# tprodanov/locityper

Hardware: AMD Instinct MI355X
Metric: reads/s through the whole genotyping path (scored + prefiltered + default solver scheme); reads_scored_per_s and genotypes_solved_per_s give the two halves (higher is better)
Workload: dtype f64

## Files before the change

locityper_amd/csrc/lcty_api.hip:

```cpp
#include <algorithm>
#include <cmath>
#include <memory>
#include <numeric>

#include "lcty_objects.hpp"

using namespace lcty;

namespace lcty {
static thread_local std::string g_last_error;
thread_local hipStream_t tl_stream = nullptr;
void set_last_error(const std::string& msg) { g_last_error = msg; }
}

hipEvent_t lcty_ctx::get_event() {
    hipEvent_t e;
    if (!event_pool.empty()) { e = event_pool.back(); event_pool.pop_back(); return e; }
    LCTY_HIP(hipEventCreate(&e));
    return e;
}

void lcty_ctx::fold_oldest(lcty::KernelTimer& t, size_t count) {
    count = std::min(count, t.pending.size());
    for (size_t i = 0; i < count; i++) {
// ... 51 lines not shown
        int n = 0;
        if (hipGetDeviceCount(&n) != hipSuccess || n == 0) {
            (void)hipGetLastError();
            fail(LCTY_ERR_RUNTIME, "no HIP device is visible: liblocityper_hip has no CPU fallback");
        }
        if (device_id < 0 || device_id >= n) fail(LCTY_ERR_INVALID_INPUT, "device %d out of range (0..%d)", device_id, n - 1);
        auto c = std::unique_ptr<lcty_ctx>(new lcty_ctx());
        c->device = device_id;
        LCTY_HIP(hipSetDevice(device_id));
        LCTY_HIP(hipGetDeviceProperties(&c->props, device_id));
        LCTY_HIP(hipStreamCreateWithFlags(&c->stream.main, hipStreamNonBlocking));
        *out = c.release();
    });
}

void lcty_ctx_destroy(lcty_ctx* ctx) {
    if (!ctx) return;
    (void)hipSetDevice(ctx->device);
    (void)hipStreamSynchronize(ctx->stream);
    for (auto& t : ctx->timers) for (auto& pr : t.pending) { (void)hipEventDestroy(pr.first); (void)hipEventDestroy(pr.second); }
    for (auto e : ctx->event_pool) (void)hipEventDestroy(e);
    if (ctx->gate.ev) (void)hipEventDestroy(ctx->gate.ev);
    if (ctx->gate.init_ev) (void)hipEventDestroy(ctx->gate.init_ev);
    if (ctx->side) { (void)hipStreamSynchronize(ctx->side); (void)hipStreamDestroy(ctx->side); }
    if (ctx->fore) { (void)hipStreamSynchronize(ctx->fore); (void)hipStreamDestroy(ctx->fore); }
    for (auto& slot : ctx->given_slots) if (slot->stream) { (void)hipStreamSynchronize(slot->stream); (void)hipStreamDestroy(slot->stream); }
    (void)hipStreamDestroy(ctx->stream.main);
    delete ctx;
}

int32_t lcty_ctx_synchronize(lcty_ctx* ctx) {
    return guarded([&] {
        if (!ctx) fail(LCTY_ERR_INVALID_INPUT, "null argument");
        ctx->activate();
        LCTY_HIP(hipStreamSynchronize(ctx->stream));
        if (ctx->side) LCTY_HIP(hipStreamSynchronize(ctx->side));
    });
}

int32_t lcty_host_alloc(lcty_ctx* ctx, uint64_t bytes, void** out) {
    return guarded([&] {
        if (!ctx || !out) fail(LCTY_ERR_INVALID_INPUT, "null argument");
        ctx->activate();
        *out = nullptr;
        LCTY_HIP(hipHostMalloc(out, std::max<uint64_t>(bytes, 1), hipHostMallocDefault));
    });
// ... 290 lines not shown
```

locityper_amd/csrc/lcty_common.hpp:

```cpp
#pragma once

#include <hip/hip_runtime.h>

#include <cstdarg>
#include <cstdint>
#include <cstdio>
#include <cstring>
#include <map>
#include <memory>
#include <condition_variable>
#include <mutex>
#include <stdexcept>
#include <string>
#include <vector>

#include "../../include/locityper_hip.h"

namespace lcty {

#ifdef LCTY_DIAG
constexpr bool kDiag = true;
#else
constexpr bool kDiag = false;
#endif
// ... 129 lines not shown
        if (!on) on = stream;
        lcty::KernelTimer& t = timers[kernel];
        hipEvent_t a, b;
        {
            std::lock_guard<std::mutex> g(timing_mutex);
            if (t.pending.size() >= 256) fold_oldest(t, 128);
            a = get_event(); b = get_event();
        }
        LCTY_HIP(hipEventRecord(a, on));
        fn();
        LCTY_HIP(hipEventRecord(b, on));
        std::lock_guard<std::mutex> g(timing_mutex);
        t.pending.emplace_back(a, b);
    }
    hipStream_t side = nullptr;
    struct LaunchGate {
        std::mutex m; std::condition_variable cv;
        uint64_t epoch = 0;
        uint64_t target = 0;
        hipEvent_t ev = nullptr;
        uint64_t tails_started = 0;
        uint64_t tail_inits = 0;
        hipEvent_t init_ev = nullptr;
    } gate;
    hipStream_t side_stream() {
        if (!side) LCTY_HIP(hipStreamCreateWithFlags(&side, hipStreamNonBlocking));
        return side;
    }
    hipStream_t fore = nullptr;
    hipStream_t fore_stream() {
        if (!fore) LCTY_HIP(hipStreamCreateWithFlags(&fore, hipStreamNonBlocking));
        return fore;
    }
    hipStream_t copy = nullptr;
    std::mutex copy_mutex;
    std::mutex ws_mutex;
    hipStream_t copy_stream() {
        std::lock_guard<std::mutex> lock(copy_mutex);
        if (!copy) LCTY_HIP(hipStreamCreateWithFlags(&copy, hipStreamNonBlocking));
        return copy;
    }
    struct SolveWorkspace {
        lcty::DevBuf<lcty::ChainRec> recs; lcty::DevBuf<lcty::ExtraLoc> extra;
        uint32_t extra_cap = 0, extra_for_ploidy = 0;
        lcty::DevBuf<uint16_t> gt; lcty::DevBuf<uint8_t> cgc; lcty::DevBuf<uint32_t> cdepth, cnnt, cseg, ctotw, ovf, cuc; lcty::DevBuf<uint64_t> seeds;
        lcty::DevBuf<double> pri, liks, parts, cww, caln, dbg;
// ... 36 lines not shown
```

locityper_amd/csrc/lcty_solve_device.hpp:

```cpp
#pragma once
#include "lcty_objects.hpp"

namespace lcty {

constexpr uint32_t MAXP = 4;
constexpr uint32_t NONE32S = 0xFFFFFFFFu;
constexpr uint32_t MID_NONE24 = 0xFFFFFFu;
constexpr uint64_t WINDOW_KEY_XOR = 0xD1B54A32D192ED03ull;
constexpr uint64_t INIT_KEY_XOR = 0x8CB92BA72F3D8DD7ull;

struct FastDiv {
    uint32_t d, m, s1, s2;
    __host__ static FastDiv make(uint32_t d) {
        FastDiv f{d, 0, 0, 0};
        uint32_t l = 0;
        while ((1ull << l) < d) l++;
        f.m = static_cast<uint32_t>(((1ull << 32) * ((1ull << l) - d)) / d + 1);
        f.s1 = l < 1 ? l : 1; f.s2 = l > 0 ? l - 1 : 0;
        return f;
    }
    __device__ __forceinline__ uint32_t div(uint32_t n) const {
        const uint32_t t = __umulhi(m, n);
        return (t + ((n - t) >> s1)) >> s2;
    }
// ... 150 lines not shown
void ensure_depth_table(lcty_locus* loc, uint64_t want);
void build_depth_table_into(const lcty_locus* loc, uint32_t depth, DevBuf<double>& out, hipStream_t s);
bool solver_lds_fits(uint32_t wstride);
struct InitHost {
    const uint16_t* genotypes; const uint64_t* seeds; const uint16_t* row_of; const lcty_locus* loc; uint32_t n_cus;
    uint32_t lds_budget;
};
void plan_init_groups(const SolveView& V, const InitHost& H, uint32_t nch, InitPlan& plan);
void launch_init(lcty_ctx* ctx, const SolveView& V, uint32_t nch, size_t lds_init, hipStream_t s, const InitHost* host, lcty_ctx::SolveWorkspace& ws,
                 InitPlan& plan);
void launch_greedy_chains(lcty_ctx* ctx, SolveView& V, uint32_t nch, hipStream_t stream, lcty_ctx::SolveWorkspace& ws);
void launch_anneal(lcty_ctx* ctx, const SolveView& V, uint32_t nch, hipStream_t s);
void launch_pause(hipStream_t s);
void launch_store_cur(ChainRec* recs, const uint32_t* words, uint64_t n, hipStream_t s);
void launch_pack_rows_count(uint64_t n, const LocCell* table, uint64_t ngp, uint32_t n_good, const uint16_t* alleles, uint32_t n_rows,
                            unsigned long long* total, hipStream_t s);
void launch_pack_rows(uint64_t n, const LocCell* table, const uint32_t* table_ext, const double* table_unm, uint64_t ngp, uint32_t n_good,
                      const uint16_t* alleles, uint32_t n_rows, const PairAlnDev* pa, LocEntry* cells, uint64_t out_stride, PairAlnDev* extras,
                      unsigned long long* cursor, hipStream_t s);
void launch_place_rows(uint64_t n, const LocEntry* cells, uint64_t in_stride, uint32_t n_good, uint32_t n_rows, uint32_t ext_base, LocCell* full,
                       uint32_t* full_ext, double* full_unm, bool write_unm, uint64_t full_stride, uint64_t first, hipStream_t s);
void launch_pad_rows(uint64_t n, LocCell* full, uint32_t* full_ext, double* full_unm, uint64_t full_stride, uint64_t from, uint32_t n_rows, hipStream_t s);
void launch_count_unexplained(uint32_t blocks, const uint8_t* status, const double* unmapped, const double* matrix, uint64_t n_pairs, uint32_t A,
                              const uint16_t* ids, uint32_t ploidy, unsigned long long* out, hipStream_t s);
void launch_read_nw(const SolveView& V, uint32_t* nw, hipStream_t s);
void launch_assignment_counts(const SolveView& V, const uint32_t* nw, const uint64_t* read_off, uint16_t* counts, hipStream_t s);

}
```

locityper_amd/csrc/lcty_solve_host.hip:

```cpp
#include <algorithm>
#include <atomic>
#include <chrono>
#include <cmath>
#include <exception>
#include <memory>
#include <numeric>
#include <future>
#include <thread>
#include <type_traits>

#include "lcty_exact.hpp"
#include "lcty_solve_device.hpp"

using namespace lcty;

namespace {

double students_t_cdf(double freedom, double x) {
    if (std::isinf(freedom)) return 0.5 * std::erfc(-x / std::sqrt(2.0));
    const double h = freedom / (freedom + x * x);
    const double ib = 0.5 * math::beta_reg(freedom / 2.0, 0.5, h);
    return x <= 0.0 ? ib : 1.0 - ib;
}

double compare_two(double mean1, double var1, uint32_t att1, double mean2, double var2, uint32_t att2) {
    const double simple_norm = mean1 - math::ln_add(mean1, mean2);
    if (std::isnormal(var1) && std::isnormal(var2)) {
// ... 16 lines not shown

void sort_by_mean(const double* lik_mean, uint64_t* ixs, uint64_t n) {
    std::sort(ixs, ixs + n, [&](uint64_t a, uint64_t b) {
        if (lik_mean[a] != lik_mean[b]) return lik_mean[a] > lik_mean[b];
        return a < b;
    });
}

double ln_sum(const double* v, size_t n) {
    if (n == 0) return -std::numeric_limits<double>::infinity();
    if (n == 1) return v[0];
    double m = -std::numeric_limits<double>::infinity();
    for (size_t i = 0; i < n; i++) m = std::fmax(m, v[i]);
    if (std::isinf(m)) return m;
    double s = 0.0;
    for (size_t i = 0; i < n; i++) s += std::exp(v[i] - m);
    return m + std::log(s);
}

}

namespace {

struct StageRunner {
    lcty_reads* reads; lcty_ctx* ctx; lcty_locus* loc;
    SolveView V{};
    uint64_t n_gt; uint32_t ploidy, attempts;
    size_t lds_init = 0;
    uint64_t gt_per_batch = 1, depth_cap = 2;
    uint32_t lane;
    hipStream_t stream;
    lcty_ctx::SolveWorkspace& ws;
    InitPlan init_plan;
    InitHost init_host{nullptr, nullptr, nullptr, nullptr, 0, 0};
    const RowGatherer* gathered_rows = nullptr;

    StageRunner(lcty_reads* r, const uint16_t* genotypes, uint64_t n_gt_, uint32_t ploidy_, const lcty_solver* solver, uint32_t attempts_,
                const uint64_t* chain_seeds, uint32_t lane_ = 0, const RowGatherer* gathered = nullptr)
        : reads(r), n_gt(n_gt_), ploidy(ploidy_), attempts(attempts_), lane(lane_), ws(check_args(r, genotypes, solver, chain_seeds, lane_)) {
        if (!reads->scored) fail(LCTY_ERR_INVALID_INPUT, "lcty_score_reads has not been called on this batch");
        if (ploidy == 0 || ploidy > MAXP) fail(LCTY_ERR_UNSUPPORTED, "the device solver handles ploidy 1..%u", MAXP);
        if (attempts == 0) fail(LCTY_ERR_INVALID_INPUT, "At least one attempt is required for each stage");
        check_solver(solver);
        ctx = reads->ctx; loc = reads->locus; gathered_rows = gathered;
        ctx->activate();
        stream = lane ? ctx->side_stream() : ctx->stream;
        reads->check_device_error(stream);
        const uint32_t A = loc->n_alleles;
        for (uint64_t i = 0; i < n_gt * ploidy; i++)
            if (genotypes[i] >= A) fail(LCTY_ERR_INVALID_INPUT, "genotype refers to allele %u >= %u", genotypes[i], A);
        if (n_gt * attempts >= 0x7FFFFFFFull) fail(LCTY_ERR_UNSUPPORTED, "too many chains in one stage");
        if (!gathered) ensure_solver_tables(reads);
        reads->stat_chains = reads->stat_iterations = reads->stat_accepted = 0;
        const uint64_t n_good = gathered ? gathered->n_good : reads->n_good_cached, ngp = gathered ? gathered->ngp : reads->ngp;
        uint32_t min_w = 0xFFFFFFFFu;
        for (uint32_t a = 0; a < A; a++) min_w = std::min(min_w, std::max(loc->n_windows[a], 1u));
        depth_cap = 2 * n_good + 2;
        uint64_t first_width = std::min<uint64_t>(4 * n_good / min_w + 64, depth_cap);
        if (ctx->knob("depth_table_start", 0) > 0)
            first_width = static_cast<uint64_t>(ctx->knob("depth_table_start", 0));
        ensure_depth_table(loc, first_width);

        V.by_window = FastDiv::make(loc->bg.window); V.by_tweak = FastDiv::make(2 * static_cast<uint32_t>(loc->prm.tweak) + 1);
        V.A = A; V.window = loc->bg.window; V.left_padding = loc->left_padding; V.tweak = static_cast<uint32_t>(loc->prm.tweak);
        V.min_weight = loc->prm.min_weight; V.prob_diff = loc->prm.prob_diff;
        V.depth_contrib = 1.0 + loc->prm.lik_skew; V.aln_contrib = 1.0 - loc->prm.lik_skew;
        V.n_windows = loc->d_n_windows.p; V.reg_start = loc->d_reg_start.p; V.allele_len = loc->d_allele_len.p;
        V.ci_off = loc->d_ci_off.p; V.gc = loc->d_gc.p; V.win_weight = loc->d_win_weight.p;
        V.uniq_cnt = loc->d_uniq_cnt.p; V.compl_cnt = loc->d_compl_cnt.p;
        const bool tables = loc->weight_tables_valid && !loc->has_explicit;
        V.wk = tables ? loc->d_wk.p : nullptr; V.wc = tables ? loc->d_wc.p : nullptr;
        V.n_wk = tables ? static_cast<uint32_t>(loc->d_wk.n) : 0u; V.n_wc = tables ? static_cast<uint32_t>(loc->d_wc.n) : 0u;
        V.lut = loc->d_lut_ext.p; V.lut_depth = loc->lut_ext_depth; V.lut_shift = static_cast<uint32_t>(__builtin_ctz(loc->lut_ext_depth)); V.depth_nb = loc->d_depth_nb.p; V.n_alt = loc->prm.n_alt_cn;
        V.n_good = static_cast<uint32_t>(n_good); V.ngp = ngp;
        set_rec_list(V, n_good);
        V.table = reinterpret_cast<const LocCell*>(reads->d_loc_table.p); V.table_ext = reads->d_loc_ext.p; V.table_unm = reads->d_loc_unm.p;
        V.pa = reads->d_pa.p; V.row_of = nullptr;
        if (gathered) {
            V.table = reinterpret_cast<const LocCell*>(reads->gather.table.p); V.table_ext = reads->gather.ext.p; V.table_unm = reads->gather.unm.p;
            V.pa = reads->gather.pa.p; V.row_of = reads->gather.row_of.p;
        }
        V.ploidy = ploidy; V.attempts = attempts; V.solver = *solver;
        V.wstride = (2 + ploidy * loc->max_n_windows + 3) & ~3u;
        lds_init = init_chain_lds(V.wstride);
        if (!solver_lds_fits(V.wstride))
            fail(LCTY_ERR_UNSUPPORTED, "%u windows per genotype: too many for the device solver", V.wstride);

        {
            const uint32_t guess = static_cast<uint32_t>(std::min<uint64_t>(ngp * (ploidy > 2 ? ploidy - 2 : 0) + std::max<uint64_t>(256, ngp / 64), (1u << 24) - 1));
            if (ws.extra_for_ploidy != ploidy) ws.extra_cap = 0;
            ws.extra_for_ploidy = ploidy;
            if (ctx->knob("solve_extra_start", 0) > 0) {
                if (ws.extra_cap == 0) ws.extra_cap = static_cast<uint32_t>(ctx->knob("solve_extra_start", 0));
            } else ws.extra_cap = std::max(ws.extra_cap, guess);
        }
        plan_batches();
        V.overflow = ws.ovf.p;
    }

    static lcty_ctx::SolveWorkspace& check_args(lcty_reads* r, const uint16_t* genotypes, const lcty_solver* solver, const uint64_t* chain_seeds,
                                                uint32_t lane) {
        if (!r || !genotypes || !solver || !chain_seeds) fail(LCTY_ERR_INVALID_INPUT, "null argument");
        return r->ctx->solve_ws[lane ? 1 : 0];
    }

    void plan_batches() {
        std::lock_guard<std::mutex> ws_lock(ctx->ws_mutex);
        const uint64_t ngp = V.rstride;
        const uint64_t per_chain = (ngp + ngp / 128) * sizeof(ChainRec) + static_cast<uint64_t>(ws.extra_cap) * sizeof(ExtraLoc) + static_cast<uint64_t>(V.wstride) * 21 + 64;
        size_t free_b = 0, total_b = 0;
        ctx->release_transfer_scratch();
        LCTY_HIP(hipMemGetInfo(&free_b, &total_b));
        const uint64_t held = ws.recs.n * sizeof(ChainRec) + ws.extra.n * sizeof(ExtraLoc);
        uint64_t budget = static_cast<uint64_t>(0.92 * static_cast<double>(free_b + held));
        if (ctx->knob("solve_budget_mb", 0) > 0)
            budget = static_cast<uint64_t>(ctx->knob("solve_budget_mb", 0)) << 20;
        gt_per_batch = std::max<uint64_t>(1, std::min<uint64_t>(n_gt, budget / (per_chain * attempts)));
        const uint64_t max_chains = gt_per_batch * attempts;
        hipStream_t s = stream;
        ws.ovf.ensure(2); ws.ovf.zero(s);
// ... 3 lines not shown
                        lane, static_cast<unsigned long long>(max_chains), static_cast<unsigned long long>(ngp), ws.recs.n * 32e-9, ws.extra.n * 16e-9,
                        free_b * 1e-9, budget * 1e-9, ws.extra_cap);
            uint64_t want_recs = std::max<uint64_t>(ws.recs.n, max_chains * (ngp + ngp / 128));
            uint64_t want_extra = std::max<uint64_t>(ws.extra.n, max_chains * static_cast<uint64_t>(ws.extra_cap) + 2);
            if (want_recs * sizeof(ChainRec) + want_extra * sizeof(ExtraLoc) > budget) {
                want_recs = max_chains * (ngp + ngp / 128); want_extra = max_chains * static_cast<uint64_t>(ws.extra_cap) + 2;
            }
            ws.recs.release(); ws.extra.release();
            ws.recs.alloc(want_recs); ws.extra.alloc(want_extra);
        }
        ws.cww.ensure(max_chains * V.wstride); ws.cgc.ensure(max_chains * V.wstride); ws.cdepth.ensure(max_chains * V.wstride);
        ws.cuc.ensure(max_chains * V.wstride);
        ws.cnnt.ensure(max_chains); ws.cseg.ensure(4 * max_chains); ws.ctotw.ensure(max_chains); ws.caln.ensure(max_chains);
        ws.gt.ensure(gt_per_batch * ploidy); ws.seeds.ensure(max_chains); ws.liks.ensure(max_chains); ws.parts.ensure(4 * max_chains);
        ws.pri.ensure(gt_per_batch);
        V.genotypes = ws.gt.p; V.seeds = ws.seeds.p; V.priors = nullptr;
        V.recs = ws.recs.p; V.extra = ws.extra.p; V.extra_cap = ws.extra_cap; V.liks = ws.liks.p; V.parts = ws.parts.p;
        V.c_ww = ws.cww.p; V.c_uc = ws.cuc.p; V.c_gc = ws.cgc.p; V.c_depth = ws.cdepth.p; V.c_nnt = ws.cnnt.p; V.c_seg = ws.cseg.p; V.c_totw = ws.ctotw.p; V.c_aln = ws.caln.p;
    }

    void upload_genotypes(const uint16_t* genotypes, uint64_t ng) { ws.gt.upload(genotypes, ng * ploidy, stream); }

    void launch(uint32_t nch) {
        if (lane == 0) wait_for_tail_init();
        launch_init(ctx, V, nch, lds_init, stream, init_host.genotypes ? &init_host : nullptr, ws, init_plan);
        if (lane == 1) announce_tail_init();
        if (V.solver.kind == LCTY_SOLVER_EXACT) { solve_exact_batch(nch); return; }
        if (V.solver.kind == LCTY_SOLVER_ANNEAL) {
            if (lane == 1) wait_for_greedy_of_next_locus();
            const bool timed_anneal = ctx->diag_knob("solve_anneal_timing", 0) != 0;
            V.dbg = nullptr;
            if (timed_anneal) { ws.dbg.ensure(12 * static_cast<size_t>(nch)); ws.dbg.zero(stream); V.dbg = ws.dbg.p; }
            launch_anneal(ctx, V, nch, stream);
            if (timed_anneal) {
                std::vector<double> d(12 * static_cast<size_t>(nch));
                ws.dbg.download(d.data(), d.size(), stream);
                LCTY_HIP(hipStreamSynchronize(stream));
                double sum[10] = {0}; size_t used = 0;
                for (size_t c = 0; c < nch; c++) if (d[12 * c + 6] > 0) { used++; for (int k = 0; k < 6; k++) sum[k] += d[12 * c + k] / d[12 * c + 6]; for (int k = 6; k < 10; k++) sum[k] += d[12 * c + k]; }
                if (used) fprintf(stderr, "[lcty anneal phases] %zu chains; second loop: %.0f rounds, %.1f moves per round, accepted %.0f of %.0f moves in all; ticks per round: wait for the ring + words %.0f, "
                                          "moves from the ring %.0f, depths + gathers + score %.0f, ballots + chain walk %.0f, apply + retire %.0f; loop total per round %.0f\n",
                                  used, sum[6] / used, sum[7] / std::max(sum[6], 1.0), sum[8] / used, sum[9] / used, sum[0] / used, sum[1] / used, sum[2] / used, sum[3] / used, sum[4] / used, sum[5] / used);
            }
            if (ctx->diag_knob("queue_trace", 0)) fprintf(stderr, "[lcty queue] %.3f ms batch %p annealing launched (lane %u)\n",
                std::chrono::duration<double, std::milli>(std::chrono::steady_clock::now().time_since_epoch()).count(), static_cast<const void*>(reads), lane);
            return;
        }
        if (lane == 0) announce_greedy();
        if (ctx->diag_knob("queue_trace", 0)) fprintf(stderr, "[lcty queue] %.3f ms batch %p greedy about to launch (lane %u)\n",
// ... 156 lines not shown
                const uint32_t c1 = shared_model ? std::min(c0 + attempts, nch) : c0 + 1;
                for (uint32_t c = c0; c < c1; c++) {
                    if (nnt[c] != h.model.n) fail(LCTY_ERR_RUNTIME, "exact solver: the attempts of a genotype without a tweak differ in their models");
                    launch_store_cur(V.recs + static_cast<uint64_t>(c) * V.rstride, d_words.p, V.rstride, s);
                    liks[c] = pri[c / attempts] + h.res.value;
                    parts[4ull * c] = h.res.aln_lik; parts[4ull * c + 1] = h.res.depth_lik; parts[4ull * c + 2] = static_cast<double>(h.res.nodes); parts[4ull * c + 3] = 0.0;
                }
                LCTY_HIP(hipStreamSynchronize(s));
            }
            LCTY_HIP(hipStreamSynchronize(s));
        }
        ws.liks.upload(liks.data(), nch, s);
        ws.parts.upload(parts.data(), 4ull * nch, s);
        LCTY_HIP(hipStreamSynchronize(s));
    }

    template <typename F>
    void run(const uint16_t* genotypes, const double* priors, const uint64_t* chain_seeds, F&& after_batch) {
        hipStream_t s = stream;
        std::vector<double> liks(gt_per_batch * attempts);
        for (uint64_t g0 = 0; g0 < n_gt;) {
            const uint64_t ng = std::min(gt_per_batch, n_gt - g0), nch = ng * attempts;
            bool smaller_batches = false;
            upload_genotypes(genotypes + g0 * ploidy, ng);
            ws.seeds.upload(chain_seeds + g0 * attempts, nch, s);
            init_host = InitHost{genotypes + g0 * ploidy, chain_seeds + g0 * attempts, gathered_rows ? gathered_rows->row_of.data() : nullptr, loc,
                                 static_cast<uint32_t>(ctx->props.multiProcessorCount), lane == 1 ? 32u * 1024u : 0u};
            if (priors) ws.pri.upload(priors + g0, ng, s);
            V.priors = priors ? ws.pri.p : nullptr;
            for (;;) {
                V.lut = loc->d_lut_ext.p; V.lut_depth = loc->lut_ext_depth; V.lut_shift = static_cast<uint32_t>(__builtin_ctz(loc->lut_ext_depth));
                launch(static_cast<uint32_t>(nch));
                uint32_t ovf[2] = {0, 0};
                ws.ovf.download(ovf, 2, s);
                ws.liks.download(liks.data(), nch, s);
                LCTY_HIP(hipStreamSynchronize(s));
                if (!ovf[0]) {
                    std::vector<double> parts(4 * nch);
                    ws.parts.download(parts.data(), 4 * nch, s);
                    LCTY_HIP(hipStreamSynchronize(s));
                    double sum = 0, mx = 0, mn = 1e300, acc = 0;
                    for (uint64_t c = 0; c < nch; c++) {
                        const double it = parts[4 * c + 2];
                        sum += it; mx = std::max(mx, it); mn = std::min(mn, it); acc += parts[4 * c + 3];
                    }
                    reads->stat_chains += nch; reads->stat_iterations += static_cast<uint64_t>(sum);
// ... 15 lines not shown
                    V.priors = priors ? ws.pri.p : nullptr;
                    if (ctx->diag_knob("queue_trace", 0))
                        fprintf(stderr, "[lcty queue] lane %u: %u further locations per chain, room for %llu genotypes a batch (had %llu)\n", lane, ws.extra_cap,
                                static_cast<unsigned long long>(gt_per_batch), static_cast<unsigned long long>(before));
                    if (gt_per_batch < ng) { smaller_batches = true; break; }
                    continue;
                }
                if (loc->lut_ext_depth >= depth_cap) fail(LCTY_ERR_RUNTIME, "window depth beyond 2 * reads + 2");
                ensure_depth_table(loc, std::min<uint64_t>(4ull * loc->lut_ext_depth, depth_cap));
            }
            if (smaller_batches) continue;
            after_batch(g0, ng, liks.data());
            g0 += ng;
        }
    }
};

}

namespace {

void solve_stage_on(uint32_t lane, lcty_reads* reads, const uint16_t* genotypes, uint64_t n_gt, uint32_t ploidy, const double* priors,
                    const lcty_solver* solver, uint32_t attempts, const uint64_t* chain_seeds, double* lik_mean, double* lik_var,
                    double* liks_out) {
    if (!lik_mean || !lik_var) fail(LCTY_ERR_INVALID_INPUT, "null argument");
    StageRunner R(reads, genotypes, n_gt, ploidy, solver, attempts, chain_seeds, lane);
    R.run(genotypes, priors, chain_seeds, [&](uint64_t g0, uint64_t ng, const double* liks) {
        for (uint64_t g = 0; g < ng; g++) {
            const double* l = liks + g * attempts;
            math::mean_variance_or_nan(l, attempts, &lik_mean[g0 + g], &lik_var[g0 + g]);
            if (liks_out) memcpy(liks_out + (g0 + g) * attempts, l, sizeof(double) * attempts);
        }
    });
}

}

RowGatherer::RowGatherer(lcty_reads* owner_, const uint16_t* genotypes, uint64_t n_gt, uint32_t ploidy) : owner(owner_) {
    if (!owner || !genotypes) fail(LCTY_ERR_INVALID_INPUT, "null argument");
    ctx = owner->ctx; ctx->activate(); stream = ctx->stream;
    const uint32_t A = owner->locus->n_alleles;
    row_of.assign(A, 0xFFFF);
    for (uint64_t i = 0; i < n_gt * ploidy; i++) {
        if (genotypes[i] >= A) fail(LCTY_ERR_INVALID_INPUT, "genotype refers to allele %u >= %u", genotypes[i], A);
        row_of[genotypes[i]] = 0;
    }
    for (uint32_t a = 0; a < A; a++)
        if (row_of[a] == 0) { row_of[a] = static_cast<uint16_t>(alleles.size()); alleles.push_back(static_cast<uint16_t>(a)); }
    n_rows = static_cast<uint32_t>(alleles.size());
// ... 299 lines not shown
        if (weighted_dist) *weighted_dist = all_known ? sum_dist / sum_prob : std::numeric_limits<double>::quiet_NaN();
    });
}

int32_t lcty_stages_default(lcty_stage* stages, uint32_t* n_stages) {
    return guarded([&] {
        if (!stages || !n_stages) fail(LCTY_ERR_INVALID_INPUT, "null argument");
        memset(stages, 0, 2 * sizeof(lcty_stage));
        lcty_solver_default(&stages[0].solver, LCTY_SOLVER_GREEDY); stages[0].in_size = 5000; stages[0].attempts = 1;
        lcty_solver_default(&stages[1].solver, LCTY_SOLVER_ANNEAL); stages[1].in_size = 20; stages[1].attempts = 20;
        *n_stages = 2;
    });
}

}

namespace {

struct LocusRun {
    lcty_reads* reads = nullptr; uint32_t ploidy = 2; const lcty_stage* stages = nullptr; uint32_t n_stages = 0;
    uint64_t master_seed = 0; const double* priors = nullptr; lcty_call* out = nullptr;
    uint64_t G = 0, n = 0, threads = 1;
    std::vector<uint16_t> gts; std::vector<uint64_t> ixs; std::vector<double> mean, var; std::vector<uint32_t> att;

    static void ok(int32_t rc) { if (rc != LCTY_OK) throw Error(rc, std::string(lcty_last_error())); }
    void mark(const char* what) const {
        if (!reads || reads->ctx->diag_knob("queue_trace", 0) == 0) return;
        const double t = std::chrono::duration<double, std::milli>(std::chrono::steady_clock::now().time_since_epoch()).count();
        fprintf(stderr, "[lcty queue] %.3f ms batch %p %s\n", t, static_cast<const void*>(reads), what);
    }

    void stage(uint32_t si, uint32_t lane) {
        const bool last = si + 1 == n_stages;
        const lcty_params& prm = reads->locus->prm;
        const uint64_t out_size = last ? 0 : stages[si + 1].in_size;
        if (!(prm.dont_skip || last || out_size < n)) return;
        const uint32_t attempts = stages[si].attempts;
        std::vector<uint16_t> sub(n * ploidy); std::vector<double> pri(n), m(n), v(n); std::vector<uint64_t> seeds(n * attempts);
        for (uint64_t t = 0; t < n; t++) {
            memcpy(sub.data() + t * ploidy, gts.data() + ixs[t] * ploidy, ploidy * sizeof(uint16_t));
            pri[t] = priors ? priors[ixs[t]] : 0.0;
        }
        ok(lcty_chain_seeds(master_seed + static_cast<uint64_t>(si + 1) * 0x9e3779b97f4a7c15ull, n * attempts, seeds.data()));
        mark(lane ? "tail stage: inputs ready" : "head stage: inputs ready");
        solve_stage_on(lane, reads, sub.data(), n, ploidy, pri.data(), &stages[si].solver, attempts, seeds.data(), m.data(), v.data(), nullptr);
        mark(lane ? "tail stage: chains done" : "head stage: chains done");
        for (uint64_t t = 0; t < n; t++) { mean[ixs[t]] = m[t]; var[ixs[t]] = v[t]; att[ixs[t]] = attempts; }
        if (!last) ok(lcty_discard_improbable(mean.data(), var.data(), att.data(), ixs.data(), n, prm.prob_thresh, out_size, threads, &n));
        mark(lane ? "tail stage: discarded" : "head stage: discarded");
    }

    void pre(bool score) {
        if (!reads || !stages || !out || n_stages == 0) fail(LCTY_ERR_INVALID_INPUT, "null argument");
        mark("head: start");
        if (score) ok(lcty_score_reads(reads));
        mark("head: scoring launched");
        if (!reads->scored) fail(LCTY_ERR_INVALID_INPUT, "lcty_score_reads has not been called on this batch");
        for (uint32_t s = 0; s < n_stages; s++)
            if (stages[s].attempts == 0 || stages[s].in_size == 0) fail(LCTY_ERR_INVALID_INPUT, "stage %u: attempts and in_size must be positive", s);
        const lcty_locus* loc = reads->locus;
        const lcty_params& prm = loc->prm;
        const uint32_t A = loc->n_alleles;
        G = count_genotypes(A, ploidy);
        gts.resize(G * ploidy);
        ok(lcty_generate_genotypes(A, ploidy, gts.data(), G));
        ixs.resize(G);
        std::iota(ixs.begin(), ixs.end(), 0ull);
        n = G;
// ... 7 lines not shown
            } else {
                std::vector<double> scores(G);
                ok(lcty_prefilter(reads, nullptr, G, ploidy, priors, scores.data()));
                ok(lcty_truncate(scores.data(), ixs.data(), G, prm.filt_diff, stages[0].in_size, threads, &n));
            }
        }
        out->kept_after_filter = n;
        mark("head: prefiltered and truncated");
        mean.assign(G, std::numeric_limits<double>::quiet_NaN()); var.assign(G, std::numeric_limits<double>::quiet_NaN());
        att.assign(G, 0);
        ensure_solver_tables(reads);
        mark("head: location table built");
    }
    void chains() { for (uint32_t si = 0; si + 1 < n_stages; si++) stage(si, 0); }
    void head(bool score) { pre(score); chains(); }

    void tail(uint32_t lane) {
        lcty_ctx* ctx = reads->ctx;
        ctx->activate();
        std::unique_ptr<StreamScope> on_side;
        if (lane) on_side = std::make_unique<StreamScope>(ctx->side_stream());
        const lcty_params& prm = reads->locus->prm;
        mark("tail: start");
        stage(n_stages - 1, lane);
        ok(lcty_produce_result(mean.data(), var.data(), att.data(), ixs.data(), n, prm.prob_thresh, 0, out->ixs, out->ln_probs, &out->n_out,
                               &out->quality));
        out->unexpl_reads = count_unexplained_on(lane ? ctx->side_stream() : ctx->stream, reads, gts.data() + out->ixs[0] * ploidy, ploidy);
        out->n_good = reads->n_good_cached;
        std::vector<uint16_t> res(out->n_out * ploidy);
        for (uint64_t t = 0; t < out->n_out; t++) memcpy(res.data() + t * ploidy, gts.data() + out->ixs[t] * ploidy, ploidy * sizeof(uint16_t));
        ok(lcty_call_checks(res.data(), out->n_out, ploidy, out->ln_probs, static_cast<uint32_t>(std::min<uint64_t>(out->n_good, 0xFFFFFFFFull)),
                            nullptr, reads->locus->n_alleles, nullptr, nullptr, &out->warnings));
    }
};

}

extern "C" {

int32_t lcty_solve(lcty_reads* reads, uint32_t ploidy, const lcty_stage* stages, uint32_t n_stages, uint64_t master_seed,
                   const double* priors, lcty_call* out, double* lik_mean_out, double* lik_var_out, uint32_t* attempts_out) {
    return guarded([&] {
        LocusRun R;
        R.reads = reads; R.ploidy = ploidy; R.stages = stages; R.n_stages = n_stages; R.master_seed = master_seed; R.priors = priors; R.out = out;
        R.head(false);
        R.tail(0);
        if (lik_mean_out) memcpy(lik_mean_out, R.mean.data(), R.G * sizeof(double));
        if (lik_var_out) memcpy(lik_var_out, R.var.data(), R.G * sizeof(double));
        if (attempts_out) memcpy(attempts_out, R.att.data(), R.G * sizeof(uint32_t));
    });
}

}

namespace {
template <typename GET, typename DONE>
void run_queue(uint32_t n, GET&& batch_of, DONE&& done_with, uint32_t ploidy, const lcty_stage* stages, uint32_t n_stages,
               const uint64_t* master_seeds, const double* const* priors, lcty_call* out) {
    std::unique_ptr<LocusRun> prev, next;
    std::thread tail_thread, fore_thread;
    int32_t tail_rc = LCTY_OK; std::string tail_msg;
    int32_t fore_rc = LCTY_OK; std::string fore_msg;
    std::shared_future<void> tail_ended;
    lcty_ctx* ctx = nullptr;
    uint32_t tail_of = 0;
    auto release_gate = [&] {
        if (!ctx) return;
        { std::lock_guard<std::mutex> lock(ctx->gate.m); if (ctx->gate.target > ctx->gate.epoch) ctx->gate.epoch = ctx->gate.target; }
        ctx->gate.cv.notify_all();
    };
    std::mutex held_mutex;
    std::vector<uint32_t> held;
    auto give_back = [&](uint32_t i) {
        { std::lock_guard<std::mutex> lock(held_mutex); held.erase(std::remove(held.begin(), held.end(), i), held.end()); }
        done_with(i);
    };
    auto join_tail = [&] {
        const bool had = tail_thread.joinable();
        if (had) tail_thread.join();
        prev.reset();
        if (tail_rc != LCTY_OK) { const int32_t rc = tail_rc; tail_rc = LCTY_OK; fail(rc, "%s", tail_msg.c_str()); }
        if (had) give_back(tail_of);
    };
    auto join_fore = [&] {
        if (fore_thread.joinable()) fore_thread.join();
        if (fore_rc != LCTY_OK) { const int32_t rc = fore_rc; fore_rc = LCTY_OK; next.reset(); fail(rc, "%s", fore_msg.c_str()); }
    };
    auto make_run = [&](uint32_t i) {
        auto R = std::make_unique<LocusRun>();
        R->reads = batch_of(i);
        { std::lock_guard<std::mutex> lock(held_mutex); held.push_back(i); }
        R->ploidy = ploidy; R->stages = stages; R->n_stages = n_stages; R->master_seed = master_seeds[i];
        R->priors = priors ? priors[i] : nullptr; R->out = &out[i];
        return R;
    };
    try {
        for (uint32_t i = 0; i < n; i++) {
            std::unique_ptr<LocusRun> R;
            if (fore_thread.joinable()) { join_fore(); R = std::move(next); }
            else { R = make_run(i); R->pre(true); }
            ctx = R->reads->ctx;
            if (i + 1 < n && ctx->knob("queue_early_head", 1) != 0) {
                std::shared_future<void> before = tail_ended;
                lcty_ctx* c = ctx;
                fore_thread = std::thread([&next, &make_run, i, before, c, &fore_rc, &fore_msg] {
                    try {
                        if (before.valid()) before.wait();
                        c->activate();
                        next = make_run(i + 1);
                        if (next->reads->ctx != c) fail(LCTY_ERR_INVALID_INPUT, "the batches of a queue share one context");
                        LocusRun* nx = next.get();
                        StreamScope on_fore(c->fore_stream());
                        nx->pre(true);
                        LCTY_HIP(hipStreamSynchronize(c->fore_stream()));
                    }
                    catch (const Error& e) { fore_rc = e.code; fore_msg = e.what(); }
                    catch (const std::exception& e) { fore_rc = LCTY_ERR_RUNTIME; fore_msg = e.what(); }
                });
            }
            try { R->chains(); }
            catch (...) { release_gate(); throw; }
            release_gate();
            join_tail();
            prev = std::move(R);
            LocusRun* run = prev.get();
            {
                std::lock_guard<std::mutex> lock(ctx->gate.m);
                ctx->gate.target = i + 1 < n && n_stages > 1 && stages[0].solver.kind == LCTY_SOLVER_GREEDY ? ctx->gate.epoch + 1 : 0;
            }
            tail_of = i;
            auto ended = std::make_shared<std::promise<void>>();
            tail_ended = ended->get_future().share();
            { std::lock_guard<std::mutex> lock(ctx->gate.m); ctx->gate.tails_started++; }
            lcty_ctx* c = ctx;
            struct StartGuard {
                lcty_ctx* c; bool armed = true;
                ~StartGuard() {
                    if (!armed) return;
                    { std::lock_guard<std::mutex> lock(c->gate.m); c->gate.tail_inits = c->gate.tails_started; }
                    c->gate.cv.notify_all();
                }
            } start_guard{c};
            tail_thread = std::thread([run, ended, c, &tail_rc, &tail_msg] {
                try { run->tail(1); }
                catch (const Error& e) { tail_rc = e.code; tail_msg = e.what(); }
                catch (const std::exception& e) { tail_rc = LCTY_ERR_RUNTIME; tail_msg = e.what(); }
                { std::lock_guard<std::mutex> lock(c->gate.m); if (c->gate.tail_inits < c->gate.tails_started) c->gate.tail_inits = c->gate.tails_started; }
                c->gate.cv.notify_all();
                ended->set_value();
            });
            start_guard.armed = false;
        }
        join_tail();
    } catch (...) {
        release_gate();
        if (fore_thread.joinable()) fore_thread.join();
        if (tail_thread.joinable()) tail_thread.join();
        if (ctx) {
            (void)hipStreamSynchronize(ctx->stream.main);
            if (ctx->side) (void)hipStreamSynchronize(ctx->side);
            if (ctx->fore) (void)hipStreamSynchronize(ctx->fore);
        }
        std::vector<uint32_t> left;
        { std::lock_guard<std::mutex> lock(held_mutex); left.swap(held); }
        for (uint32_t i : left) {
            try { done_with(i); } catch (...) {}
        }
        throw;
    }
}
}

// ... 98 lines not shown
```

locityper_amd/csrc/lcty_solve_kernels.hip:

```cpp
#include <algorithm>
#include <cmath>
#include <type_traits>
#include <vector>

#include "lcty_solve_device.hpp"

namespace lcty {


__global__ __launch_bounds__(256) void build_loc_table_kernel(const uint32_t* __restrict__ good_ix, uint32_t n_good, uint64_t ngp,
                                                              uint32_t A, const uint32_t* __restrict__ pa_idx,
                                                              const uint64_t* __restrict__ pa_off, const PairAlnDev* __restrict__ pa,
                                                              const double* __restrict__ unmapped, LocCell* __restrict__ table,
                                                              uint32_t* __restrict__ table_ext, double* __restrict__ table_unm,
                                                              uint32_t* __restrict__ err) {
    __shared__ LocCell tile[32][33];
    __shared__ uint32_t tile_ext[32][33];
    const uint32_t g0 = blockIdx.x * 32, c0 = blockIdx.y * 32;
    const uint32_t tx = threadIdx.x & 31u, ty = threadIdx.x >> 5;
    if (blockIdx.y == 0 && threadIdx.x < 32) {
        const uint32_t g = g0 + threadIdx.x;
        if (g < ngp) table_unm[g] = g < n_good ? unmapped[good_ix[g]] : 0.0;
    }
    for (uint32_t i = ty; i < 32; i += 8) {
// ... 1570 lines not shown
            d[5] = static_cast<double>(__builtin_amdgcn_s_memtime() - t_first); d[6] = static_cast<double>(n_rounds); d[7] = static_cast<double>(n_walked);
            d[8] = static_cast<double>(n_acc); d[9] = static_cast<double>(n_iter);
        }
    }
    if (!handed_over) __syncthreads();
    __hip_atomic_store(&ring->stop, 1u, __ATOMIC_RELAXED, __HIP_MEMORY_SCOPE_WORKGROUP);
    if (lane == 0) {
        const double lik = V.depth_contrib * depth_lik + V.aln_contrib * aln_lik;
        V.liks[chain] = (V.priors ? V.priors[gi] : 0.0) + lik;
        V.parts[4 * chain] = aln_lik; V.parts[4 * chain + 1] = depth_lik; V.parts[4 * chain + 2] = static_cast<double>(n_iter);
        V.parts[4 * chain + 3] = static_cast<double>(n_acc);
    }
}

__global__ __launch_bounds__(256) void store_cur_kernel(ChainRec* __restrict__ recs, const uint32_t* __restrict__ words, uint64_t n) {
    const uint64_t i = static_cast<uint64_t>(blockIdx.x) * 256 + threadIdx.x;
    if (i < n) recs[i].rp_cur = words[i];
}

__global__ __launch_bounds__(256) void count_unexplained_kernel(const uint8_t* __restrict__ status, const double* __restrict__ unmapped,
                                                                const double* __restrict__ matrix, uint64_t n_pairs, uint32_t A,
                                                                const uint16_t* __restrict__ ids, uint32_t ploidy,
                                                                unsigned long long* __restrict__ out) {
    uint32_t mine = 0;
    for (uint64_t r = blockIdx.x * 256ull + threadIdx.x; r < n_pairs; r += static_cast<uint64_t>(gridDim.x) * 256ull) {
        if (status[r] != LCTY_READ_GOOD) continue;
        double best = -INFINITY;
        for (uint32_t i = 0; i < ploidy; i++) best = fmax(best, matrix[r * A + ids[i]]);
        mine += best < unmapped[r] + 1e-8;
    }
    const unsigned long long bal = __ballot(mine != 0);
    if (bal) {
        for (int o = 32; o > 0; o >>= 1) mine += __shfl_xor(static_cast<int>(mine), o);
        if ((threadIdx.x & 63u) == 0) atomicAdd(out, static_cast<unsigned long long>(mine));
    }
}

template <uint32_t P>
__global__ __launch_bounds__(256) void read_nw_kernel(const SolveView V, uint32_t* __restrict__ nw) {
    const uint32_t g = blockIdx.x * 256 + threadIdx.x;
    if (g >= V.n_good) return;
    Geno<P> G; G.init(V, 0);
    Locs<P> L; locs_init(L, V, g, G);
    nw[g] = L.nw;
}

// ... 300 lines not shown
void launch_pack_rows_count(uint64_t n, const LocCell* table, uint64_t ngp, uint32_t n_good, const uint16_t* alleles, uint32_t n_rows,
                            unsigned long long* total, hipStream_t s) {
    hipLaunchKernelGGL(pack_rows_count_kernel, dim3(static_cast<uint32_t>((n + 255) / 256)), dim3(256), 0, s, table, ngp, n_good, alleles, n_rows, total);
    LCTY_HIP(hipGetLastError());
}
void launch_pack_rows(uint64_t n, const LocCell* table, const uint32_t* table_ext, const double* table_unm, uint64_t ngp, uint32_t n_good,
                      const uint16_t* alleles, uint32_t n_rows, const PairAlnDev* pa, LocEntry* cells, uint64_t out_stride, PairAlnDev* extras,
                      unsigned long long* cursor, hipStream_t s) {
    hipLaunchKernelGGL(pack_rows_kernel, dim3(static_cast<uint32_t>((n + 255) / 256)), dim3(256), 0, s, table, table_ext, table_unm, ngp, n_good, alleles,
                       n_rows, pa, cells, out_stride, extras, cursor);
    LCTY_HIP(hipGetLastError());
}
void launch_place_rows(uint64_t n, const LocEntry* cells, uint64_t in_stride, uint32_t n_good, uint32_t n_rows, uint32_t ext_base, LocCell* full,
                       uint32_t* full_ext, double* full_unm, bool write_unm, uint64_t full_stride, uint64_t first, hipStream_t s) {
    hipLaunchKernelGGL(place_rows_kernel, dim3(static_cast<uint32_t>((n + 255) / 256)), dim3(256), 0, s, cells, in_stride, n_good, n_rows, ext_base, full,
                       full_ext, full_unm, write_unm, full_stride, first);
    LCTY_HIP(hipGetLastError());
}
void launch_pad_rows(uint64_t n, LocCell* full, uint32_t* full_ext, double* full_unm, uint64_t full_stride, uint64_t from, uint32_t n_rows, hipStream_t s) {
    hipLaunchKernelGGL(pad_rows_kernel, dim3(static_cast<uint32_t>((n + 255) / 256)), dim3(256), 0, s, full, full_ext, full_unm, full_stride, from, n_rows);
    LCTY_HIP(hipGetLastError());
}
void launch_count_unexplained(uint32_t blocks, const uint8_t* status, const double* unmapped, const double* matrix, uint64_t n_pairs, uint32_t A,
                              const uint16_t* ids, uint32_t ploidy, unsigned long long* out, hipStream_t s) {
    hipLaunchKernelGGL(count_unexplained_kernel, dim3(blocks), dim3(256), 0, s, status, unmapped, matrix, n_pairs, A, ids, ploidy, out);
    LCTY_HIP(hipGetLastError());
}
void launch_read_nw(const SolveView& V, uint32_t* nw, hipStream_t s) {
    if (!V.n_good) return;
    const uint32_t blocks = (V.n_good + 255) / 256;
    switch (V.ploidy) {
        case 1: hipLaunchKernelGGL(read_nw_kernel<1>, dim3(blocks), dim3(256), 0, s, V, nw); break;
        case 2: hipLaunchKernelGGL(read_nw_kernel<2>, dim3(blocks), dim3(256), 0, s, V, nw); break;
        case 3: hipLaunchKernelGGL(read_nw_kernel<3>, dim3(blocks), dim3(256), 0, s, V, nw); break;
        default: hipLaunchKernelGGL(read_nw_kernel<4>, dim3(blocks), dim3(256), 0, s, V, nw); break;
    }
    LCTY_HIP(hipGetLastError());
}
void launch_assignment_counts(const SolveView& V, const uint32_t* nw, const uint64_t* read_off, uint16_t* counts, hipStream_t s) {
    if (!V.n_good) return;
    hipLaunchKernelGGL(assignment_counts_kernel, dim3((V.n_good + 255) / 256), dim3(256), 0, s, V, nw, read_off, counts);
    LCTY_HIP(hipGetLastError());
}

}
```

Measured before the change: 2.622 million.

## Release read batch to next locus head once last tail stage initialises

Adds a BatchLease so the next locus's head stage can take the shared read buffers as soon as the final anneal stage of the current tail has initialised its last batch. Previously it had to wait for the whole tail thread to finish. To allow this, unexplained-read counts for all remaining genotypes (up to 64) are computed ahead of time with a 2D-grid count kernel before the buffers are released. The final call then looks up its count instead of re-reading the matrix after the solve. This adds cross-thread lease and event logic, re-binding of batch pointers, and extra counting work for genotypes that are not chosen.

```diff
diff --git a/locityper_amd/csrc/lcty_api.hip b/locityper_amd/csrc/lcty_api.hip
--- a/locityper_amd/csrc/lcty_api.hip
+++ b/locityper_amd/csrc/lcty_api.hip
@@ -97,6 +97,7 @@
     for (auto e : ctx->event_pool) (void)hipEventDestroy(e);
     if (ctx->gate.ev) (void)hipEventDestroy(ctx->gate.ev);
     if (ctx->gate.init_ev) (void)hipEventDestroy(ctx->gate.init_ev);
+    for (auto e : ctx->gate.free_ev) if (e) (void)hipEventDestroy(e);
     if (ctx->side) { (void)hipStreamSynchronize(ctx->side); (void)hipStreamDestroy(ctx->side); }
     if (ctx->fore) { (void)hipStreamSynchronize(ctx->fore); (void)hipStreamDestroy(ctx->fore); }
     for (auto& slot : ctx->given_slots) if (slot->stream) { (void)hipStreamSynchronize(slot->stream); (void)hipStreamDestroy(slot->stream); }
diff --git a/locityper_amd/csrc/lcty_common.hpp b/locityper_amd/csrc/lcty_common.hpp
--- a/locityper_amd/csrc/lcty_common.hpp
+++ b/locityper_amd/csrc/lcty_common.hpp
@@ -175,6 +175,7 @@
         uint64_t tails_started = 0;
         uint64_t tail_inits = 0;
         hipEvent_t init_ev = nullptr;
+        hipEvent_t free_ev[2] = {nullptr, nullptr};
     } gate;
     hipStream_t side_stream() {
         if (!side) LCTY_HIP(hipStreamCreateWithFlags(&side, hipStreamNonBlocking));
diff --git a/locityper_amd/csrc/lcty_solve_device.hpp b/locityper_amd/csrc/lcty_solve_device.hpp
--- a/locityper_amd/csrc/lcty_solve_device.hpp
+++ b/locityper_amd/csrc/lcty_solve_device.hpp
@@ -196,7 +196,7 @@
                        uint32_t* full_ext, double* full_unm, bool write_unm, uint64_t full_stride, uint64_t first, hipStream_t s);
 void launch_pad_rows(uint64_t n, LocCell* full, uint32_t* full_ext, double* full_unm, uint64_t full_stride, uint64_t from, uint32_t n_rows, hipStream_t s);
 void launch_count_unexplained(uint32_t blocks, const uint8_t* status, const double* unmapped, const double* matrix, uint64_t n_pairs, uint32_t A,
-                              const uint16_t* ids, uint32_t ploidy, unsigned long long* out, hipStream_t s);
+                              const uint16_t* ids, uint32_t ploidy, unsigned long long* out, hipStream_t s, uint32_t n_genotypes = 1);
 void launch_read_nw(const SolveView& V, uint32_t* nw, hipStream_t s);
 void launch_assignment_counts(const SolveView& V, const uint32_t* nw, const uint64_t* read_off, uint16_t* counts, hipStream_t s);
 
diff --git a/locityper_amd/csrc/lcty_solve_host.hip b/locityper_amd/csrc/lcty_solve_host.hip
--- a/locityper_amd/csrc/lcty_solve_host.hip
+++ b/locityper_amd/csrc/lcty_solve_host.hip
@@ -3,6 +3,7 @@
 #include <chrono>
 #include <cmath>
 #include <exception>
+#include <functional>
 #include <memory>
 #include <numeric>
 #include <future>
@@ -65,6 +66,52 @@
 
 namespace {
 
+struct BatchLease {
+    std::mutex m; std::condition_variable cv;
+    bool free = false;
+    bool taken = false;
+    bool head_done = false;
+    bool head_failed = false;
+    bool recorded = false;
+    hipEvent_t ev = nullptr;
+    uint64_t greedy_target = 0;
+    bool reclaim() {
+        std::unique_lock<std::mutex> lock(m);
+        if (!free) return false;
+        if (!taken) { free = false; return false; }
+        cv.wait(lock, [&] { return head_done; });
+        if (head_failed) fail(LCTY_ERR_RUNTIME, "the stage has to be initialised again, and the head of a later position failed on what may be its batch");
+        return true;
+    }
+    void release(hipStream_t s) {
+        LCTY_HIP(hipEventRecord(ev, s));
+        { std::lock_guard<std::mutex> lock(m); recorded = true; free = true; }
+        cv.notify_all();
+    }
+    void ended() {
+        { std::lock_guard<std::mutex> lock(m); free = true; }
+        cv.notify_all();
+    }
+    void take(hipStream_t s) {
+        bool wait_ev;
+        {
+            std::unique_lock<std::mutex> lock(m);
+            cv.wait(lock, [&] { return free; });
+            taken = true; wait_ev = recorded;
+        }
+        if (wait_ev) LCTY_HIP(hipStreamWaitEvent(s, ev, 0));
+    }
+    void head_ended(bool ok) {
+        { std::lock_guard<std::mutex> lock(m); head_done = true; head_failed = !ok; }
+        cv.notify_all();
+    }
+};
+
+struct StageHooks {
+    std::function<bool()> before_init;
+    std::function<void(bool)> after_init;
+};
+
 struct StageRunner {
     lcty_reads* reads; lcty_ctx* ctx; lcty_locus* loc;
     SolveView V{};
@@ -77,6 +124,8 @@
     InitPlan init_plan;
     InitHost init_host{nullptr, nullptr, nullptr, nullptr, 0, 0};
     const RowGatherer* gathered_rows = nullptr;
+    const StageHooks* hooks = nullptr;
+    bool last_batch = false;
 
     StageRunner(lcty_reads* r, const uint16_t* genotypes, uint64_t n_gt_, uint32_t ploidy_, const lcty_solver* solver, uint32_t attempts_,
                 const uint64_t* chain_seeds, uint32_t lane_ = 0, const RowGatherer* gathered = nullptr)
@@ -117,12 +166,7 @@
         V.lut = loc->d_lut_ext.p; V.lut_depth = loc->lut_ext_depth; V.lut_shift = static_cast<uint32_t>(__builtin_ctz(loc->lut_ext_depth)); V.depth_nb = loc->d_depth_nb.p; V.n_alt = loc->prm.n_alt_cn;
         V.n_good = static_cast<uint32_t>(n_good); V.ngp = ngp;
         set_rec_list(V, n_good);
-        V.table = reinterpret_cast<const LocCell*>(reads->d_loc_table.p); V.table_ext = reads->d_loc_ext.p; V.table_unm = reads->d_loc_unm.p;
-        V.pa = reads->d_pa.p; V.row_of = nullptr;
-        if (gathered) {
-            V.table = reinterpret_cast<const LocCell*>(reads->gather.table.p); V.table_ext = reads->gather.ext.p; V.table_unm = reads->gather.unm.p;
-            V.pa = reads->gather.pa.p; V.row_of = reads->gather.row_of.p;
-        }
+        bind_batch();
         V.ploidy = ploidy; V.attempts = attempts; V.solver = *solver;
         V.wstride = (2 + ploidy * loc->max_n_windows + 3) & ~3u;
         lds_init = init_chain_lds(V.wstride);
@@ -139,6 +183,15 @@
         }
         plan_batches();
         V.overflow = ws.ovf.p;
+    }
+
+    void bind_batch() {
+        V.table = reinterpret_cast<const LocCell*>(reads->d_loc_table.p); V.table_ext = reads->d_loc_ext.p; V.table_unm = reads->d_loc_unm.p;
+        V.pa = reads->d_pa.p; V.row_of = nullptr;
+        if (gathered_rows) {
+            V.table = reinterpret_cast<const LocCell*>(reads->gather.table.p); V.table_ext = reads->gather.ext.p; V.table_unm = reads->gather.unm.p;
+            V.pa = reads->gather.pa.p; V.row_of = reads->gather.row_of.p;
+        }
     }
 
     static lcty_ctx::SolveWorkspace& check_args(lcty_reads* r, const uint16_t* genotypes, const lcty_solver* solver, const uint64_t* chain_seeds,
@@ -188,9 +241,11 @@
     void upload_genotypes(const uint16_t* genotypes, uint64_t ng) { ws.gt.upload(genotypes, ng * ploidy, stream); }
 
     void launch(uint32_t nch) {
+        if (hooks && hooks->before_init && hooks->before_init()) bind_batch();
         if (lane == 0) wait_for_tail_init();
         launch_init(ctx, V, nch, lds_init, stream, init_host.genotypes ? &init_host : nullptr, ws, init_plan);
         if (lane == 1) announce_tail_init();
+        if (hooks && hooks->after_init) hooks->after_init(last_batch);
         if (V.solver.kind == LCTY_SOLVER_EXACT) { solve_exact_batch(nch); return; }
         if (V.solver.kind == LCTY_SOLVER_ANNEAL) {
             if (lane == 1) wait_for_greedy_of_next_locus();
@@ -393,6 +448,7 @@
         for (uint64_t g0 = 0; g0 < n_gt;) {
             const uint64_t ng = std::min(gt_per_batch, n_gt - g0), nch = ng * attempts;
             bool smaller_batches = false;
+            last_batch = g0 + ng == n_gt;
             upload_genotypes(genotypes + g0 * ploidy, ng);
             ws.seeds.upload(chain_seeds + g0 * attempts, nch, s);
             init_host = InitHost{genotypes + g0 * ploidy, chain_seeds + g0 * attempts, gathered_rows ? gathered_rows->row_of.data() : nullptr, loc,
@@ -454,9 +510,10 @@
 
 void solve_stage_on(uint32_t lane, lcty_reads* reads, const uint16_t* genotypes, uint64_t n_gt, uint32_t ploidy, const double* priors,
                     const lcty_solver* solver, uint32_t attempts, const uint64_t* chain_seeds, double* lik_mean, double* lik_var,
-                    double* liks_out) {
+                    double* liks_out, const StageHooks* hooks = nullptr) {
     if (!lik_mean || !lik_var) fail(LCTY_ERR_INVALID_INPUT, "null argument");
     StageRunner R(reads, genotypes, n_gt, ploidy, solver, attempts, chain_seeds, lane);
+    R.hooks = hooks;
     R.run(genotypes, priors, chain_seeds, [&](uint64_t g0, uint64_t ng, const double* liks) {
         for (uint64_t g = 0; g < ng; g++) {
             const double* l = liks + g * attempts;
@@ -802,6 +859,9 @@
     uint64_t master_seed = 0; const double* priors = nullptr; lcty_call* out = nullptr;
     uint64_t G = 0, n = 0, threads = 1;
     std::vector<uint16_t> gts; std::vector<uint64_t> ixs; std::vector<double> mean, var; std::vector<uint32_t> att;
+    BatchLease* lease = nullptr;
+    std::vector<unsigned long long> unexpl_all;
+    static constexpr uint64_t MAX_COUNTED_AHEAD = 64;
 
     static void ok(int32_t rc) { if (rc != LCTY_OK) throw Error(rc, std::string(lcty_last_error())); }
     void mark(const char* what) const {
@@ -823,7 +883,33 @@
         }
         ok(lcty_chain_seeds(master_seed + static_cast<uint64_t>(si + 1) * 0x9e3779b97f4a7c15ull, n * attempts, seeds.data()));
         mark(lane ? "tail stage: inputs ready" : "head stage: inputs ready");
-        solve_stage_on(lane, reads, sub.data(), n, ploidy, pri.data(), &stages[si].solver, attempts, seeds.data(), m.data(), v.data(), nullptr);
+        StageHooks hooks;
+        const bool let_go = last && lease && stages[si].solver.kind == LCTY_SOLVER_ANNEAL && n <= MAX_COUNTED_AHEAD;
+        if (let_go) {
+            lcty_ctx* ctx = reads->ctx;
+            const hipStream_t s = lane ? ctx->side_stream() : static_cast<hipStream_t>(ctx->stream);
+            reads->d_unexpl_ids.ensure(MAX_COUNTED_AHEAD * MAXP); reads->d_unexpl_out.ensure(MAX_COUNTED_AHEAD);
+            hooks.before_init = [this] { return lease->reclaim(); };
+            hooks.after_init = [this, &sub, s](bool last_batch) {
+                if (!last_batch) return;
+                reads->d_unexpl_ids.upload(sub.data(), n * ploidy, s);
+                reads->d_unexpl_out.zero(s);
+                const uint32_t blocks = static_cast<uint32_t>(std::min<uint64_t>((reads->n_pairs + 255) / 256, 4096));
+                if (reads->n_pairs)
+                    launch_count_unexplained(blocks, reads->d_status.p, reads->d_unmapped.p, reads->d_matrix.p, reads->n_pairs, reads->locus->n_alleles,
+                                             reads->d_unexpl_ids.p, ploidy, reads->d_unexpl_out.p, s, static_cast<uint32_t>(n));
+                lease->release(s);
+                mark("tail stage: batch free");
+            };
+        }
+        solve_stage_on(lane, reads, sub.data(), n, ploidy, pri.data(), &stages[si].solver, attempts, seeds.data(), m.data(), v.data(), nullptr,
+                       let_go ? &hooks : nullptr);
+        if (let_go) {
+            const hipStream_t s = lane ? reads->ctx->side_stream() : static_cast<hipStream_t>(reads->ctx->stream);
+            unexpl_all.resize(n);
+            reads->d_unexpl_out.download(unexpl_all.data(), n, s);
+            LCTY_HIP(hipStreamSynchronize(s));
+        }
         mark(lane ? "tail stage: chains done" : "head stage: chains done");
         for (uint64_t t = 0; t < n; t++) { mean[ixs[t]] = m[t]; var[ixs[t]] = v[t]; att[ixs[t]] = attempts; }
         if (!last) ok(lcty_discard_improbable(mean.data(), var.data(), att.data(), ixs.data(), n, prm.prob_thresh, out_size, threads, &n));
@@ -877,11 +963,15 @@
         if (lane) on_side = std::make_unique<StreamScope>(ctx->side_stream());
         const lcty_params& prm = reads->locus->prm;
         mark("tail: start");
+        const uint64_t n_good = reads->n_good_cached;
         stage(n_stages - 1, lane);
         ok(lcty_produce_result(mean.data(), var.data(), att.data(), ixs.data(), n, prm.prob_thresh, 0, out->ixs, out->ln_probs, &out->n_out,
                                &out->quality));
-        out->unexpl_reads = count_unexplained_on(lane ? ctx->side_stream() : ctx->stream, reads, gts.data() + out->ixs[0] * ploidy, ploidy);
-        out->n_good = reads->n_good_cached;
+        if (unexpl_all.empty())
+            out->unexpl_reads = count_unexplained_on(lane ? ctx->side_stream() : ctx->stream, reads, gts.data() + out->ixs[0] * ploidy, ploidy);
+        else
+            out->unexpl_reads = static_cast<uint32_t>(unexpl_all[static_cast<size_t>(std::find(ixs.begin(), ixs.begin() + n, out->ixs[0]) - ixs.begin())]);
+        out->n_good = n_good;
         std::vector<uint16_t> res(out->n_out * ploidy);
         for (uint64_t t = 0; t < out->n_out; t++) memcpy(res.data() + t * ploidy, gts.data() + out->ixs[t] * ploidy, ploidy * sizeof(uint16_t));
         ok(lcty_call_checks(res.data(), out->n_out, ploidy, out->ln_probs, static_cast<uint32_t>(std::min<uint64_t>(out->n_good, 0xFFFFFFFFull)),
@@ -916,7 +1006,7 @@
     std::thread tail_thread, fore_thread;
     int32_t tail_rc = LCTY_OK; std::string tail_msg;
     int32_t fore_rc = LCTY_OK; std::string fore_msg;
-    std::shared_future<void> tail_ended;
+    std::shared_ptr<BatchLease> tail_lease;
     lcty_ctx* ctx = nullptr;
     uint32_t tail_of = 0;
     auto release_gate = [&] {
@@ -956,18 +1046,26 @@
             else { R = make_run(i); R->pre(true); }
             ctx = R->reads->ctx;
             if (i + 1 < n && ctx->knob("queue_early_head", 1) != 0) {
-                std::shared_future<void> before = tail_ended;
+                std::shared_ptr<BatchLease> before = tail_lease;
                 lcty_ctx* c = ctx;
                 fore_thread = std::thread([&next, &make_run, i, before, c, &fore_rc, &fore_msg] {
+                    struct Through { BatchLease* l; bool ok = false; ~Through() { if (l) l->head_ended(ok); } } through{before.get()};
                     try {
-                        if (before.valid()) before.wait();
                         c->activate();
+                        if (before) {
+                            before->take(c->fore_stream());
+                            auto& g = c->gate;
+                            std::unique_lock<std::mutex> lock(g.m);
+                            g.cv.wait(lock, [&] { return g.epoch >= before->greedy_target; });
+                            if (before->greedy_target && g.ev) LCTY_HIP(hipStreamWaitEvent(c->fore_stream(), g.ev, 0));
+                        }
                         next = make_run(i + 1);
                         if (next->reads->ctx != c) fail(LCTY_ERR_INVALID_INPUT, "the batches of a queue share one context");
                         LocusRun* nx = next.get();
                         StreamScope on_fore(c->fore_stream());
                         nx->pre(true);
                         LCTY_HIP(hipStreamSynchronize(c->fore_stream()));
+                        through.ok = true;
                     }
                     catch (const Error& e) { fore_rc = e.code; fore_msg = e.what(); }
                     catch (const std::exception& e) { fore_rc = LCTY_ERR_RUNTIME; fore_msg = e.what(); }
@@ -984,9 +1082,17 @@
                 ctx->gate.target = i + 1 < n && n_stages > 1 && stages[0].solver.kind == LCTY_SOLVER_GREEDY ? ctx->gate.epoch + 1 : 0;
             }
             tail_of = i;
-            auto ended = std::make_shared<std::promise<void>>();
-            tail_ended = ended->get_future().share();
-            { std::lock_guard<std::mutex> lock(ctx->gate.m); ctx->gate.tails_started++; }
+            auto lease = std::make_shared<BatchLease>();
+            {
+                std::lock_guard<std::mutex> lock(ctx->gate.m);
+                hipEvent_t& ev = ctx->gate.free_ev[i & 1u];
+                if (!ev) LCTY_HIP(hipEventCreateWithFlags(&ev, hipEventDisableTiming));
+                lease->ev = ev;
+                lease->greedy_target = ctx->gate.target;
+                ctx->gate.tails_started++;
+            }
+            tail_lease = lease;
+            run->lease = lease.get();
             lcty_ctx* c = ctx;
             struct StartGuard {
                 lcty_ctx* c; bool armed = true;
@@ -996,13 +1102,13 @@
                     c->gate.cv.notify_all();
                 }
             } start_guard{c};
-            tail_thread = std::thread([run, ended, c, &tail_rc, &tail_msg] {
+            tail_thread = std::thread([run, lease, c, &tail_rc, &tail_msg] {
                 try { run->tail(1); }
                 catch (const Error& e) { tail_rc = e.code; tail_msg = e.what(); }
                 catch (const std::exception& e) { tail_rc = LCTY_ERR_RUNTIME; tail_msg = e.what(); }
                 { std::lock_guard<std::mutex> lock(c->gate.m); if (c->gate.tail_inits < c->gate.tails_started) c->gate.tail_inits = c->gate.tails_started; }
                 c->gate.cv.notify_all();
-                ended->set_value();
+                lease->ended();
             });
             start_guard.armed = false;
         }
diff --git a/locityper_amd/csrc/lcty_solve_kernels.hip b/locityper_amd/csrc/lcty_solve_kernels.hip
--- a/locityper_amd/csrc/lcty_solve_kernels.hip
+++ b/locityper_amd/csrc/lcty_solve_kernels.hip
@@ -1616,6 +1616,7 @@
                                                                 const double* __restrict__ matrix, uint64_t n_pairs, uint32_t A,
                                                                 const uint16_t* __restrict__ ids, uint32_t ploidy,
                                                                 unsigned long long* __restrict__ out) {
+    ids += static_cast<size_t>(blockIdx.y) * ploidy; out += blockIdx.y;
     uint32_t mine = 0;
     for (uint64_t r = blockIdx.x * 256ull + threadIdx.x; r < n_pairs; r += static_cast<uint64_t>(gridDim.x) * 256ull) {
         if (status[r] != LCTY_READ_GOOD) continue;
@@ -1962,8 +1963,8 @@
     LCTY_HIP(hipGetLastError());
 }
 void launch_count_unexplained(uint32_t blocks, const uint8_t* status, const double* unmapped, const double* matrix, uint64_t n_pairs, uint32_t A,
-                              const uint16_t* ids, uint32_t ploidy, unsigned long long* out, hipStream_t s) {
-    hipLaunchKernelGGL(count_unexplained_kernel, dim3(blocks), dim3(256), 0, s, status, unmapped, matrix, n_pairs, A, ids, ploidy, out);
+                              const uint16_t* ids, uint32_t ploidy, unsigned long long* out, hipStream_t s, uint32_t n_genotypes) {
+    hipLaunchKernelGGL(count_unexplained_kernel, dim3(blocks, n_genotypes), dim3(256), 0, s, status, unmapped, matrix, n_pairs, A, ids, ploidy, out);
     LCTY_HIP(hipGetLastError());
 }
 void launch_read_nw(const SolveView& V, uint32_t* nw, hipStream_t s) {
```

Result: no change. 2.613 million (-0.3%).
